# Apokleos/kata-xpu-device-plugin

Hardware: NVIDIA H100
Metric: pci.ids parse GB/s (x1000 text + 2^20-key join); device lookups/s reported beside it (higher is better)
Workload: dtype u8

## Files before the change

kata-xpu-device-plugin_b200/csrc/api.cu:

```cuda
#include <algorithm>
#include <cstdlib>
#include <new>
#include <vector>

#include "internal.cuh"
#include "pciids5.cu"
#include "finalize.cuh"
#include "small.cuh"
#include "scan.cuh"

void kx_exchange_destroy(kxpu_ctx *ctx);

static const char *kx_err_names[] = {
    "ok", "invalid argument", "CUDA error", "no sm_90 GPU available", "output buffer too small",
    "table capacity exceeded", "NCCL / peer exchange unavailable or failed", "input outside the supported domain", "out of memory"};

extern "C" const char *kxpu_strerror(int32_t status) {
    int i = -status;
    if (i < 0 || i > 8) return "unknown status";
    return kx_err_names[i];
}

extern "C" const char *kxpu_last_error(kxpu_ctx *ctx) {
    if (!ctx) return "null ctx";
// ... 293 lines not shown
    if (!t) return;
    if (t->arena.p) {
        if (ctx->pool.size() >= 4) {
            cudaStreamSynchronize(ctx->stream);
            cudaFree(ctx->pool.front().p);
            ctx->pool.erase(ctx->pool.begin());
        }
        arena_reset(ctx, t->arena);
        ctx->pool.push_back(t->arena);
    }
    delete t;
}

uint32_t kx_initial_blob_cap(kxpu_ctx *ctx, size_t n) {
    const uint32_t by_text = (uint32_t)std::min<size_t>(std::max<size_t>(n, 256), 4u << 20);
    return ctx->blob_hint > by_text ? ctx->blob_hint : by_text;
}

bool kx_grow_cap(uint32_t *cap, bool table_full) {
    if (*cap >= (1u << 28)) return false;
    const uint32_t sh = table_full ? 4u : 2u;
    *cap = (*cap >> (28u - sh)) ? (1u << 28) : (*cap << sh);
    return true;
}

void kx_note_table_size(kxpu_ctx *ctx, uint32_t nkeys, uint32_t blob_used, uint32_t blob_cap) {
    uint32_t ideal = 1u << 16;
    while (ideal < (1u << 28) && ideal / 2 < nkeys + nkeys / 8) ideal <<= 1;
    ctx->cap_hint = ideal;
    ctx->blob_hint = blob_cap > (4u << 20) && blob_used > (2u << 20) ? blob_cap : 0u;
}

int32_t kx_launch_parse(kxpu_ctx *ctx, kxpu_table *t, const uint8_t *d_text, size_t n, unsigned long long base,
                        unsigned long long carry_in, const KxXaHook *xa) {
    using namespace kxparse;
    const uint32_t num_chunks = (uint32_t)((n + CW - 1) / CW);
    kxparse5::Params5 P;
    memset(&P, 0, sizeof P);
    if (xa) { P.xa_on = 1; P.xa_done = xa->done; P.xa = xa->p; }
    if (num_chunks == 0) {
        if (xa) {
            P.tab = t->dev;
            P.task_ctas = 0;
            kxparse5::resolve_chunks_kernel<<<kxparse5::XA_CTAS, kxparse5::RES_WARPS * 32, 0, ctx->stream>>>(P);
            KX_LAUNCHED(ctx);
            KX_CUDA(ctx, cudaGetLastError());
        }
        return KXPU_OK;
    }
    P.text = d_text; P.n = n; P.base = base; P.num_chunks = num_chunks;
    P.tma_limit = n >= (size_t)STG_BYTES ? (uint32_t)((n - STG_BYTES) / CW) + 1u : 0u;
    static int per_sm = 0;
    const size_t smem = sizeof(kxparse5::WarpSmem5) * WARPS;
    if (per_sm == 0) {
        cudaOccupancyMaxActiveBlocksPerMultiprocessor(&per_sm, kxparse5::parse_kernel_v5, NT, smem);
        if (per_sm < 1) per_sm = 1;
    }
    const uint32_t wave_warps = (uint32_t)per_sm * ctx->sm_count * WARPS;
    P.rch = std::min<uint32_t>(std::max<uint32_t>(num_chunks / (wave_warps * 8u), 1u), kxparse5::RCH5_MAX);
    if (ctx->force_rch) P.rch = (uint32_t)ctx->force_rch;
    P.num_ranges = (num_chunks + P.rch - 1) / P.rch;
    P.range_state = t->range_words;
    P.range_carry = t->range_words + P.num_ranges;
    P.lead = (uint32_t *)(t->range_words + 2 * P.num_ranges);
    P.tasks = P.lead + P.num_ranges;
    P.tab = t->dev; P.carry_in = carry_in;
    uint32_t grid = (uint32_t)per_sm * ctx->sm_count;
    const uint32_t need = (P.num_ranges + WARPS - 1) / WARPS;
    if (grid > need) grid = need;
    {
        KxTimer tm(ctx, KXPU_T_PARSE);
        kxparse5::parse_kernel_v5<<<grid, NT, smem, ctx->stream>>>(P);
        KX_LAUNCHED(ctx);
    }
    {
        KxTimer tr(ctx, KXPU_T_RESOLVE);
        kxparse5::resolve_ranges_kernel<<<(P.num_ranges + 255u) / 256u, 256, 0, ctx->stream>>>(P);
        KX_LAUNCHED(ctx);
        const uint32_t rgrid = std::min<uint32_t>(4u * ctx->sm_count, (num_chunks + kxparse5::RES_WARPS - 1) / kxparse5::RES_WARPS);
        P.task_ctas = rgrid;
        kxparse5::resolve_chunks_kernel<<<rgrid + (xa ? kxparse5::XA_CTAS : 0u), kxparse5::RES_WARPS * 32, 0, ctx->stream>>>(P);
        KX_LAUNCHED(ctx);
    }
    KX_CUDA(ctx, cudaGetLastError());
    return KXPU_OK;
}

int32_t kx_launch_trunc(kxpu_ctx *ctx, kxpu_table *t, const uint8_t *d_text, size_t n, unsigned long long base) {
    kxparse::trunc_kernel<<<1, 1024, 0, ctx->stream>>>(d_text, n, base, t->dev.trunc, t->dev.counters);
    KX_LAUNCHED(ctx);
    KX_CUDA(ctx, cudaGetLastError());
    return KXPU_OK;
}

int32_t kx_launch_finalize(kxpu_ctx *ctx, kxpu_table *t, const uint8_t *d_text, size_t n, unsigned long long base,
                           const kxx::MinView *mv, const kxx::WaitSpec *wait, const KxSlabOut *slab) {
    kxparse::FinalizeParams F;
    memset(&F, 0, sizeof F);
    if (wait) F.wait = *wait;
    F.text = d_text; F.n = n; F.base = base; F.tab = t->dev;
    if (mv) F.mv = *mv;
    else { F.mv.a = t->dev.vendor_first; F.mv.stride = 0; F.mv.n = 1; F.mv.trunc1 = t->dev.trunc; }
    F.row_key = t->row_key; F.row_line = t->row_line; F.row_anchor = t->row_anchor;
    F.row_name_off = t->row_name_off; F.row_name_len = t->row_name_len;
    F.blob = t->blob; F.blob_cap = t->blob_cap;
    if (slab) {
        F.slab_rows = reinterpret_cast<kxx::SlabRow *>(slab->rows); F.slab_rows_cap = slab->rows_cap;
        F.blob = slab->blob; F.blob_cap = slab->blob_cap;
        F.tail = slab->tail;
    }
    KxTimer tm(ctx, KXPU_T_FINALIZE);
    F.scan_w = t->cap >= (1u << 19) ? 32u : 8u;
    if (ctx->force_scan_w) F.scan_w = (uint32_t)ctx->force_scan_w;
    const unsigned batches = (t->cap + 1 + F.scan_w - 1) / F.scan_w;
    const unsigned grid = std::min<unsigned>((batches + kxparse::SF_WARPS - 1) / kxparse::SF_WARPS, 8u * ctx->sm_count);
    kxparse::select_finalize_kernel<<<grid, kxparse::SF_WARPS * 32, 0, ctx->stream>>>(F);
    KX_LAUNCHED(ctx);
    KX_CUDA(ctx, cudaGetLastError());
    return KXPU_OK;
}

int32_t kx_launch_lookup(kxpu_ctx *ctx, kxpu_table *t, const uint32_t *d_keys, size_t n, int32_t *d_rows) {
    if (n == 0) return KXPU_OK;
    KxTimer tm(ctx, KXPU_T_LOOKUP);
    size_t blocks = (n + 255) / 256;
    size_t maxb = (size_t)ctx->sm_count * 32;
    if (blocks > maxb) blocks = maxb;
    kxparse::lookup_kernel<<<(unsigned)blocks, 256, 0, ctx->stream>>>(d_keys, n, t->dev.slots, t->cap, t->shift, d_rows);
    KX_LAUNCHED(ctx);
    KX_CUDA(ctx, cudaGetLastError());
    return KXPU_OK;
}

struct KxJoin {
    const uint32_t *d_keys;
    size_t n;
    int32_t *d_rows;
    int32_t *h_rows;
    const uint8_t *src_text;
};

static void *kx_mapped_host(const void *p) {
    if (!p) return nullptr;
    cudaPointerAttributes at;
    if (cudaPointerGetAttributes(&at, p) != cudaSuccess) { cudaGetLastError(); return nullptr; }
    return at.type == cudaMemoryTypeHost ? at.devicePointer : nullptr;
}

static uint32_t small_text_chunks(kxpu_ctx *ctx) {
    if (ctx->small_chunks < 0) {
        int coop = 0, per_sm = 0;
        cudaDeviceGetAttribute(&coop, cudaDevAttrCooperativeLaunch, ctx->device);
        cudaFuncSetAttribute(kxsmall::small_load_kernel, cudaFuncAttributeMaxDynamicSharedMemorySize, kxparse::WARPS * kxparse::STG_BYTES);
        cudaOccupancyMaxActiveBlocksPerMultiprocessor(&per_sm, kxsmall::small_load_kernel, kxparse::NT, kxparse::WARPS * kxparse::STG_BYTES);
        cudaGetLastError();
        ctx->small_chunks = (coop && !ctx->no_small) ? per_sm * ctx->sm_count * kxparse::WARPS : 0;
    }
    return (uint32_t)ctx->small_chunks;
}

static int32_t launch_small(kxpu_ctx *ctx, kxpu_table *t, const uint8_t *d_text, size_t n, const KxJoin *join) {
// ... 67 lines not shown
                    const long long t1 = tf[b * 8 + k], t0 = k ? tf[b * 8 + k - 1] : h[b * 8 + 4];
                    if (!t1 || !t0) continue;
                    const long long d = t1 - t0;
                    mn = std::min(mn, d); mx = std::max(mx, d); sum += d; cnt++;
                }
                if (cnt) fprintf(stderr, " %s %lld/%lld/%lld |", fn[k], mn, sum / cnt, mx);
            }
        }
        fprintf(stderr, "\n");
    }
    return KXPU_OK;
}

static int32_t kx_build_table_join(kxpu_ctx *ctx, const uint8_t *d_text, size_t n, kxpu_table **out, const KxJoin *join) {
    if ((reinterpret_cast<uintptr_t>(d_text) & 15u) != 0) {
        KX_SET_ERR(ctx, "device text pointer must be 16-byte aligned");
        return KXPU_E_INVALID;
    }
    if (n >= (1ull << 44)) return KXPU_E_UNSUPPORTED;
    uint32_t cap = ctx->cap_hint;
    while (cap > (1u << 16) && (size_t)cap / 2 > n / 6 + 1) cap >>= 1;
    uint32_t blob_cap = kx_initial_blob_cap(ctx, n);
    const uint32_t num_chunks = (uint32_t)((n + kxparse::CW - 1) / kxparse::CW);
    bool have_trunc = false;
    for (int attempt = 0; attempt < 12; attempt++) {
        kxpu_table *t = nullptr;
        int32_t rc = kx_table_acquire(ctx, cap, blob_cap, num_chunks, &t);
        if (rc != KXPU_OK) return rc;
        const bool small_path = num_chunks > 0 && num_chunks <= small_text_chunks(ctx) && !have_trunc;
        if (small_path) {
            rc = launch_small(ctx, t, d_text, n, join);
        } else {
            if (join && join->src_text && attempt == 0) cudaMemcpyAsync(const_cast<uint8_t *>(d_text), join->src_text, n, cudaMemcpyDefault, ctx->stream);
            rc = kx_launch_parse(ctx, t, d_text, n, 0, 0, nullptr);
            if (rc == KXPU_OK && have_trunc) rc = kx_launch_trunc(ctx, t, d_text, n, 0);
            if (rc == KXPU_OK) rc = kx_launch_finalize(ctx, t, d_text, n, 0, nullptr, nullptr, nullptr);
            if (rc == KXPU_OK && join) rc = kx_launch_lookup(ctx, t, join->d_keys, join->n, join->d_rows);
        }
        if (rc != KXPU_OK) { kx_table_release(ctx, t); return rc; }
        const bool zero_copy = small_path && join && join->src_text;
        if (!zero_copy) {
            if (join && join->h_rows && join->n) cudaMemcpyAsync(join->h_rows, join->d_rows, join->n * 4, cudaMemcpyDeviceToHost, ctx->stream);
            cudaMemcpyAsync(ctx->h_ctl, t->dev.counters, KX_C_COUNT * 4, cudaMemcpyDeviceToHost, ctx->stream);
        }
        cudaError_t e = cudaStreamSynchronize(ctx->stream);
        if (e != cudaSuccess) {
            KX_SET_ERR(ctx, "parse/finalize failed: %s", cudaGetErrorString(e));
            kx_table_release(ctx, t);
            return KXPU_E_CUDA;
        }
        const uint32_t *h = ctx->h_ctl;
        if (h[KX_C_OVERFLOW] || h[KX_C_NKEYS] > t->dev.max_keys) {
            kx_table_release(ctx, t);
            if (!kx_grow_cap(&cap, h[KX_C_OVERFLOW] != 0)) return KXPU_E_CAPACITY;
            continue;
        }
        if (h[KX_C_NEED_TRUNC] == 2u) {
            kx_table_release(ctx, t);
            have_trunc = true;
            continue;
        }
        if (h[KX_C_BLOB_OVERFLOW]) {
            kx_table_release(ctx, t);
            if ((size_t)blob_cap >= n) return KXPU_E_CAPACITY;
            blob_cap = (uint32_t)std::min<size_t>(std::max<size_t>(n, 256), (size_t)blob_cap * 8);
            continue;
        }
        t->n_rows = h[KX_C_NSEL];
        t->blob_used = h[KX_C_BLOB_CURSOR];
        kx_note_table_size(ctx, h[KX_C_NKEYS], t->blob_used, blob_cap);
        *out = t;
        return KXPU_OK;
    }
    return KXPU_E_CAPACITY;
}

// ... 187 lines not shown
```

kata-xpu-device-plugin_b200/csrc/common.cuh:

```cuda
#pragma once
#include <cuda_runtime.h>
#include <stdint.h>
#include <stdio.h>
#include <string.h>

#include <mutex>
#include <vector>

#include "../../include/kxpu.h"

constexpr int KX_MAX_RANKS = 16;


struct KxArena {
    void *p = nullptr;
    size_t bytes = 0;
    uint32_t cap = 0, blob_cap = 0;
    size_t range_bytes = 0;
};

struct KxExchange;
struct kxpu_multi;

struct kxpu_ctx {
    int device = -1;
    int sm_count = 0;
    cudaStream_t stream = nullptr;
    cudaEvent_t ev[2 * KXPU_T_COUNT] = {};
    cudaEvent_t ev_user[2] = {};
    bool ev_used[KXPU_T_COUNT] = {};
    int force_rch = 0;
    bool no_small = false;
    bool no_zero_copy = false;
    int force_scan_w = 0;
    int small_chunks = -1;
    bool stage_timing = true;
    uint64_t launches = 0;
    std::mutex mu;
    char err[512] = {0};
// ... 37 lines not shown
    void stop() {
        if (open) { cudaEventRecord(c->ev[2 * idx + 1], c->stream); c->ev_used[idx] = true; open = false; }
    }
    ~KxTimer() { stop(); }
};

static inline void kx_clear_timings(kxpu_ctx *c) { memset(c->ev_used, 0, sizeof(c->ev_used)); }

unsigned long long *kx_scan_state(kxpu_ctx *ctx, size_t words);
uint32_t kx_next_epoch(kxpu_ctx *ctx);

struct KxScratch {
    kxpu_ctx *c;
    std::vector<void *> ptrs;
    explicit KxScratch(kxpu_ctx *ctx) : c(ctx) {}
    cudaError_t alloc(void **p, size_t bytes) {
        cudaError_t e = cudaMallocAsync(p, bytes ? bytes : 16, c->stream);
        if (e == cudaSuccess) ptrs.push_back(*p);
        else *p = nullptr;
        return e;
    }
    ~KxScratch() {
        for (void *p : ptrs) cudaFreeAsync(p, c->stream);
    }
};

#ifdef __CUDACC__
__device__ __forceinline__ uint32_t kx_lane() { return threadIdx.x & 31u; }

__device__ __forceinline__ void kx_fence_gpu() { asm volatile("fence.acq_rel.gpu;" ::: "memory"); }
__device__ __forceinline__ void kx_fence_sys() { asm volatile("fence.acq_rel.sys;" ::: "memory"); }

__device__ __forceinline__ uint32_t kx_hash(uint32_t key) { return key * 0x9E3779B1u; }
#endif
```

kata-xpu-device-plugin_b200/csrc/finalize.cuh:

```cuda
#pragma once
#include "exchange.cuh"
#include "parse_common.cuh"

namespace kxparse {

constexpr unsigned long long MAX_TOKEN = 65536ull;

__global__ void __launch_bounds__(1024) trunc_kernel(const uint8_t *__restrict__ text, unsigned long long n,
                                                      unsigned long long base, unsigned long long *trunc_out, uint32_t *counters) {
    __shared__ unsigned long long s_first[1024], s_last[1024], s_bad[1024];
    const unsigned long long per = (n + 1023ull) / 1024ull;
    const unsigned long long lo = per * threadIdx.x, hi = lo + per < n ? lo + per : n;
    unsigned long long first = KX_NO_OFF, last = KX_NO_OFF, bad = KX_NO_OFF;
    for (unsigned long long i = lo; i < hi; i++) {
        if (text[i] == (uint8_t)'\n') {
            if (first == KX_NO_OFF) first = i;
            else if (i - last - 1 >= MAX_TOKEN && bad == KX_NO_OFF) bad = last + 1;
            last = i;
        }
    }
    s_first[threadIdx.x] = first; s_last[threadIdx.x] = last; s_bad[threadIdx.x] = bad;
    __syncthreads();
    if (threadIdx.x == 0) {
        unsigned long long prev_nl = KX_NO_OFF;
        unsigned long long res = KX_NO_OFF;
        for (int k = 0; k < 1024 && res == KX_NO_OFF; k++) {
            if (s_first[k] != KX_NO_OFF) {
                unsigned long long start = prev_nl == KX_NO_OFF ? 0 : prev_nl + 1;
                if (s_first[k] - start >= MAX_TOKEN) { res = start; break; }
                if (s_bad[k] != KX_NO_OFF) { res = s_bad[k]; break; }
                prev_nl = s_last[k];
            }
        }
        if (res == KX_NO_OFF) {
            unsigned long long start = prev_nl == KX_NO_OFF ? 0 : prev_nl + 1;
            if (n - start >= MAX_TOKEN) res = start;
        }
        *trunc_out = res == KX_NO_OFF ? KX_NO_OFF : base + res;
        counters[KX_C_NEED_TRUNC] = 1u;
    }
}

__device__ __forceinline__ bool is_re_space(uint32_t c) {
    return c == 0x20u || c == 0x09u || c == 0x0au || c == 0x0cu || c == 0x0du;
}
__device__ __forceinline__ uint32_t uspace_len(const uint8_t *s, uint32_t len) {
    if (len == 0) return 0;
    uint32_t c = s[0];
    if (c == 0x20u || (c >= 0x09u && c <= 0x0du)) return 1;
    if (len >= 2 && c == 0xC2u && (s[1] == 0x85u || s[1] == 0xA0u)) return 2;
    if (len >= 3) {
        uint32_t d = s[1], e = s[2];
        if (c == 0xE1u && d == 0x9Au && e == 0x80u) return 3;
        if (c == 0xE2u && d == 0x80u && ((e >= 0x80u && e <= 0x8Au) || e == 0xA8u || e == 0xA9u || e == 0xAFu)) return 3;
        if (c == 0xE2u && d == 0x81u && e == 0x9Fu) return 3;
// ... 16 lines not shown
    uint32_t c = buf[i];
    if (is_re_space(c)) return (i > start && is_re_space(buf[i - 1])) ? 0u : (uint32_t)'_';
    if (c >= 'a' && c <= 'z') return c - 32u;
    if (c == '/' || c == '.') return (uint32_t)'_';
    if ((c >= 'A' && c <= 'Z') || (c >= '0' && c <= '9') || c == '_') return c;
    if (i + 1 < end) {
        if (c == 0xC4u && buf[i + 1] == 0xB1u) return (uint32_t)'I';
        if (c == 0xC5u && buf[i + 1] == 0xBFu) return (uint32_t)'S';
    }
    return 0u;
}

constexpr int SF_WARPS = 8;
constexpr int SF_WIN = 128;
constexpr int SF_BATCH = 8;

struct FinalizeParams {
    const uint8_t *text;
    unsigned long long n, base;
    KxTableDev tab;
    kxx::MinView mv;
    uint32_t *row_key;
    unsigned long long *row_line;
    unsigned long long *row_anchor;
    uint32_t *row_name_off;
    uint32_t *row_name_len;
    uint8_t *blob;
    uint32_t blob_cap;
    kxx::WaitSpec wait;
    kxx::SlabRow *slab_rows;
    uint32_t slab_rows_cap;
    uint32_t scan_w;
    kxx::SlabTail tail;
    long long *trace;
};

__device__ __forceinline__ void finalize_store_row(const FinalizeParams &F, uint32_t row, uint32_t slot, uint32_t key, unsigned long long line,
                                                   unsigned long long anchor, uint32_t name_off, uint32_t name_len) {
    F.tab.slots[slot].row = (int32_t)row;
    if (F.slab_rows) {
        if (row < F.slab_rows_cap) {
            kxx::SlabRow r;
            r.key = key; r.name_len = name_len; r.line = line; r.anchor = anchor; r.name_off = name_off; r.pad = 0u;
            F.slab_rows[row] = r;
        }
    } else {
        F.row_key[row] = key; F.row_line[row] = line; F.row_anchor[row] = anchor;
        F.row_name_off[row] = name_off; F.row_name_len[row] = name_len;
    }
}

struct SfEntry {
    unsigned long long line, anchor;
    uint32_t slot, key;
};
constexpr int SF_QCAP = SF_BATCH - 1 + 32;

#define SF_MARK(k) do { if (F.trace && threadIdx.x == 0 && F.trace[blockIdx.x * 8u + (k)] == 0) F.trace[blockIdx.x * 8u + (k)] = clock64(); } while (0)

__device__ __forceinline__ void select_finalize_body(const FinalizeParams &F, const uint32_t scan_w) {
    __shared__ __align__(16) uint8_t s_raw[SF_WARPS][4][SF_WIN + 16];
    __shared__ uint8_t s_name[SF_WARPS][SF_BATCH][SF_WIN];
    __shared__ __align__(8) SfEntry s_q[SF_WARPS][SF_QCAP + 1];
    __shared__ uint32_t s_cnt[SF_WARPS], s_bytes[SF_WARPS], s_more[SF_WARPS], s_row0, s_blob0;
    if (F.tab.counters[KX_C_LONGLINE_HINT] != 0u && F.tab.counters[KX_C_NEED_TRUNC] != 1u) {
        if (blockIdx.x == 0 && threadIdx.x == 0) F.tab.counters[KX_C_NEED_TRUNC] = 2u;
// ... 221 lines not shown
                trim_space(g, len, start, end);
                for (uint32_t i = start; i < end; i++) out_len += sanitise_byte(g, i, start, end) != 0u;
                at = out_len ? atomicAdd(&F.tab.counters[KX_C_BLOB_CURSOR], out_len) : 0u;
                if (at + out_len > F.blob_cap) { F.tab.counters[KX_C_BLOB_OVERFLOW] = 1u; ok = false; }
                if (ok) {
                    uint32_t wr = at;
                    for (uint32_t i = start; i < end; i++) {
                        const uint32_t ch = sanitise_byte(g, i, start, end);
                        if (ch) F.blob[wr++] = (uint8_t)ch;
                    }
                }
            }
            if (lane == 0) finalize_store_row(F, row0 + r, l_slot, l_key, l_line, l_anchor, ok ? at : 0u, ok ? out_len : 0u);
            __syncwarp();
        }
        SF_MARK(5);
        {
            const uint32_t rem = qn - nvalid;
            if (nvalid != 0u && rem != 0u) {
                SfEntry e;
                if (lane < rem) e = q[nvalid + lane];
                __syncwarp();
                if (lane < rem) q[lane] = e;
                __syncwarp();
            }
            qn = rem;
        }
        __syncthreads();
        SF_MARK(6);
        if (!more) break;
    }
}

__global__ void __launch_bounds__(SF_WARPS * 32, 8) select_finalize_kernel(const FinalizeParams F) {
    kxx::wait_flags_cta(F.wait);
    select_finalize_body(F, F.scan_w);
    if (F.tail.on) {
        __syncthreads();
        if (threadIdx.x == 0) {
            kx_fence_sys();
            const uint32_t prev = atomicAdd(F.tail.done, 1u);
            if (prev == gridDim.x - 1u) {
                *F.tail.done = 0u;
                kx_fence_gpu();
                const volatile uint32_t *c = F.tab.counters;
                const uint32_t n_sel = c[KX_C_NSEL], blob_used = c[KX_C_BLOB_CURSOR];
                const bool over = c[KX_C_BLOB_OVERFLOW] || n_sel > F.tail.rows_cap || blob_used > F.tail.blob_cap;
                kxx::SlabHeader h;
                memset(&h, 0, sizeof h);
                h.n_rows = over ? 0u : n_sel;
                h.blob_bytes = over ? 0u : blob_used;
                h.status = over ? kxx::XS_SLAB_OVERFLOW : 0u;
                if (c[KX_C_OVERFLOW]) h.status |= kxx::XS_GROW | kxx::XS_FULL;
                if (c[KX_C_NKEYS] > F.tab.max_keys) h.status |= kxx::XS_GROW;
                h.nkeys = c[KX_C_NKEYS];
                *F.tail.header = h;
                kx_fence_sys();
                for (int k = 0; k < F.tail.tg.n; k++) *reinterpret_cast<volatile uint32_t *>(F.tail.tg.region[k] + F.tail.o_flag) = F.tail.epoch;
            }
        }
    }
}

__global__ void __launch_bounds__(256) lookup_kernel(const uint32_t *__restrict__ keys, size_t n, const KxSlot *__restrict__ slots,
                                                      uint32_t cap, uint32_t shift, int32_t *__restrict__ rows_out) {
    size_t i = (size_t)blockIdx.x * blockDim.x + threadIdx.x;
    const size_t stride = (size_t)gridDim.x * blockDim.x;
    for (; i < n; i += stride) rows_out[i] = table_probe(slots, cap, shift, keys[i]);
}

__global__ void __launch_bounds__(256) name_len_kernel(const int32_t *__restrict__ rows, size_t n,
                                                        const uint32_t *__restrict__ row_name_len, uint32_t n_rows,
                                                        uint32_t *__restrict__ lens) {
    size_t i = (size_t)blockIdx.x * blockDim.x + threadIdx.x;
    if (i < n) {
        int32_t r = rows[i];
        lens[i] = (r >= 0 && (uint32_t)r < n_rows) ? row_name_len[r] : 0u;
    }
}
__global__ void __launch_bounds__(256) name_copy_kernel(const int32_t *__restrict__ rows, size_t n,
                                                         const uint32_t *__restrict__ row_name_off,
                                                         const uint32_t *__restrict__ row_name_len, uint32_t n_rows,
                                                         const uint8_t *__restrict__ blob,
                                                         const uint32_t *__restrict__ offsets, uint8_t *__restrict__ out,
                                                         size_t cap) {
    size_t i = ((size_t)blockIdx.x * blockDim.x + threadIdx.x) >> 3;
    uint32_t sub = threadIdx.x & 7u;
    if (i >= n) return;
    int32_t r = rows[i];
    if (r < 0 || (uint32_t)r >= n_rows) return;
    uint32_t len = row_name_len[r], src = row_name_off[r], dst = offsets[i];
    if ((size_t)dst + len > cap) return;
    for (uint32_t k = sub; k < len; k += 8u) out[dst + k] = blob[src + k];
}

__global__ void __launch_bounds__(256) arena_reset_kernel(uint4 *ff, size_t n_ff16, uint32_t *counters) {
    const size_t i = (size_t)blockIdx.x * blockDim.x + threadIdx.x;
    const size_t stride = (size_t)gridDim.x * blockDim.x;
// ... 6 lines not shown
```

kata-xpu-device-plugin_b200/csrc/internal.cuh:

```cuda
#pragma once
#include "common.cuh"
#include "exchange.cuh"
#include "table.cuh"

struct kxpu_table {
    uint32_t cap = 0, shift = 0;
    KxArena arena;
    KxTableDev dev{};
    unsigned long long *range_words = nullptr;
    uint32_t *row_key = nullptr;
    unsigned long long *row_line = nullptr;
    unsigned long long *row_anchor = nullptr;
    uint32_t *row_name_off = nullptr;
    uint32_t *row_name_len = nullptr;
    uint32_t *sel = nullptr;
    uint8_t *blob = nullptr;
    uint32_t blob_cap = 0;
    uint32_t rows_cap = 0;
    uint32_t n_rows = 0;
    uint32_t blob_used = 0;
};

#define KX_ENTER(ctx)                          \
    if (!(ctx)) return KXPU_E_INVALID;         \
    std::lock_guard<std::mutex> guard__((ctx)->mu); \
    cudaSetDevice((ctx)->device)

int32_t kx_table_acquire(kxpu_ctx *ctx, uint32_t cap, uint32_t blob_cap, uint32_t num_chunks, kxpu_table **out);
void kx_table_release(kxpu_ctx *ctx, kxpu_table *t);
uint32_t kx_initial_blob_cap(kxpu_ctx *ctx, size_t n);
struct KxXaHook {
    kxx::XaParams p;
    uint32_t *done;
};
int32_t kx_launch_parse(kxpu_ctx *ctx, kxpu_table *t, const uint8_t *d_text, size_t n, unsigned long long base,
                        unsigned long long carry_in, const KxXaHook *xa);
int32_t kx_launch_trunc(kxpu_ctx *ctx, kxpu_table *t, const uint8_t *d_text, size_t n, unsigned long long base);
struct KxSlabOut {
    uint8_t *rows;
    uint32_t rows_cap;
    uint8_t *blob;
    uint32_t blob_cap;
    kxx::SlabTail tail;
};
int32_t kx_launch_finalize(kxpu_ctx *ctx, kxpu_table *t, const uint8_t *d_text, size_t n, unsigned long long base,
                           const kxx::MinView *mv, const kxx::WaitSpec *wait, const KxSlabOut *slab);
int32_t kx_launch_lookup(kxpu_ctx *ctx, kxpu_table *t, const uint32_t *d_keys, size_t n, int32_t *d_rows);
bool kx_grow_cap(uint32_t *cap, bool table_full);
void kx_note_table_size(kxpu_ctx *ctx, uint32_t nkeys, uint32_t blob_used, uint32_t blob_cap);
```

kata-xpu-device-plugin_b200/csrc/pciids5.cu:

```cuda
#pragma once
#include "exchange.cuh"
#include "parse_common.cuh"

namespace kxparse5 {

using namespace kxparse;

constexpr int STAGES5 = 3;
constexpr int RCH5_MAX = 8;
constexpr int RES_WARPS = 8;

struct WarpSmem5 {
    alignas(16) uint8_t stage[STAGES5][STG_BYTES];
    alignas(8) unsigned long long bar[STAGES5];
};

struct Params5 {
    const uint8_t *text;
    unsigned long long n, base;
    uint32_t num_chunks;
    uint32_t tma_limit;
    uint32_t rch;
    uint32_t num_ranges;
    unsigned long long *range_state;
    uint32_t *lead;
    unsigned long long *range_carry;
    uint32_t *tasks;
    KxTableDev tab;
    unsigned long long carry_in;
    uint32_t task_ctas;
    int xa_on;
    uint32_t *xa_done;
    kxx::XaParams xa;
};


__device__ __forceinline__ void nl_masks(uint32_t st, uint32_t lane, uint32_t n_rel, uint32_t k7f, uint32_t k0a, uint32_t k80,
                                         uint32_t (&nl)[2], uint32_t &rawnl) {
    const uint32_t swz = (lane >> 2) & 1u;
    rawnl = 0;
#pragma unroll
    for (int h = 0; h < 2; h++) {
        const uint32_t o = (uint32_t)h * HALF + lane * 32u;
        const uint4 va = lds128(st + o + 16u * swz);
        const uint4 vb = lds128(st + o + 16u * (swz ^ 1u));
        const uint32_t ma = nl_mask16(va, k7f, k0a, k80), mb = nl_mask16(vb, k7f, k0a, k80);
        const uint32_t m2 = ma | (mb << 16);
        uint32_t mm = __funnelshift_l(m2, m2, swz << 4);
        rawnl |= mm;
        if (n_rel <= (uint32_t)CW) mm &= n_rel > o + 1u ? (n_rel - o - 1u >= 32u ? 0xffffffffu : ((1u << (n_rel - o - 1u)) - 1u)) : 0u;
        nl[h] = mm;
    }
}

// ... 17 lines not shown
        const uint32_t c0 = lds8(lp0 + (31u - (uint32_t)__clz((int)b0)));
        const uint32_t c1 = lds8(lp0 + (uint32_t)HALF + (31u - (uint32_t)__clz((int)b1)));
        if (c0 != 9u && c0 != 35u) t0 |= b0;
        if (c1 != 9u && c1 != 35u) t1 |= b1;
    }
}

__device__ __forceinline__ uint32_t devs_of(uint32_t lp, uint32_t mm) {
    uint32_t km = 0;
    while (mm) {
        const uint32_t bit = mm & (0u - mm);
        mm ^= bit;
        const uint32_t a = lp + (31u - (uint32_t)__clz((int)bit));
        if (lds8(a) == 9u && lds8(a + 1u) != 9u) km |= bit;
    }
    return km;
}

__global__ void __launch_bounds__(NT, 4) parse_kernel_v5(const Params5 P) {
    extern __shared__ __align__(128) uint8_t smem_raw[];
    WarpSmem5 *W = reinterpret_cast<WarpSmem5 *>(smem_raw);
    uint32_t lane = threadIdx.x & 31u;
    const uint32_t w = threadIdx.x >> 5;
    asm volatile("" : "+r"(lane));
    const uint32_t lt_mask = (1u << lane) - 1u;

    if (lane == 0) {
        for (int s = 0; s < STAGES5; s++) mbar_init(&W[w].bar[s], 1);
        asm volatile("fence.mbarrier_init.release.cluster;" ::: "memory");
    }
    uint32_t tk = 0;
    if (lane == 0) tk = atomicAdd(&P.tab.counters[KX_C_TICKET], 1u);
    uint32_t r = __shfl_sync(0xffffffffu, tk, 0);
    if (r >= P.num_ranges) return;

    uint32_t a_stage0 = smem_u32(smem_raw) + w * (uint32_t)sizeof(WarpSmem5);
    asm volatile("" : "+r"(a_stage0));
    const uint32_t a_bar0 = a_stage0 + (uint32_t)offsetof(WarpSmem5, bar);

    uint32_t k7f = 0x7f7f7f7fu, k0a = 0x0a0a0a0au, k80 = 0x80808080u;
    asm volatile("" : "+r"(k7f), "+r"(k0a), "+r"(k80));

    const unsigned long long pol = l2_evict_first_policy();
    auto issue = [&](uint32_t g, uint32_t s) {
        if (g < P.tma_limit) {
            mbar_expect_tx_a(a_bar0 + 8u * s, STG_BYTES);
            tma_load_a(a_stage0 + s * (uint32_t)STG_BYTES, P.text + (unsigned long long)g * CW, STG_BYTES, a_bar0 + 8u * s, pol);
        }
    };
    const uint32_t rch = P.rch;
    bool staged = false;

    uint32_t phase_bits = 0, s = 0;
    uint32_t nfresh = 0;
    for (;;) {
        uint32_t tk2 = 0, r_next = 0xffffffffu;
        bool have_next = false;
        if (lane == 0) tk2 = atomicAdd(&P.tab.counters[KX_C_TICKET], 1u);
        uint32_t rc_x = 0, rc_g = 0;
        if (r == 0u) {
            rc_x = LS_PUB | (((P.carry_in & CV_HAS_TOP) && (P.carry_in & CV_VOK)) ? (LS_TOP | LS_VOK) : 0u);
            rc_g = 0xffffffffu;
        }
        uint32_t lead = r == 0u ? 0u : rch;
        const bool table_dead = *reinterpret_cast<volatile uint32_t *>(&P.tab.counters[KX_C_OVERFLOW]) != 0u;
        const uint32_t gb = r * rch;
        const uint32_t cnt = P.num_chunks - gb < rch ? P.num_chunks - gb : rch;
        if (!staged && lane == 0) {
            for (uint32_t j = 0; j < (uint32_t)STAGES5 && j < cnt; j++) issue(gb + j, (s + j) % (uint32_t)STAGES5);
        }
        staged = false;
        for (uint32_t i = 0; i < cnt; i++) {
            if (!have_next && rch > (uint32_t)STAGES5 && i + (uint32_t)STAGES5 >= rch) {
                r_next = __shfl_sync(0xffffffffu, tk2, 0);
                have_next = true;
            }
            const uint32_t g = gb + i;
            const uint32_t st = a_stage0 + s * (uint32_t)STG_BYTES;
            const unsigned long long cbase = P.base + (unsigned long long)g * CW;
            uint32_t n_rel = CW + 1;
            if (g < P.tma_limit) {
                const uint32_t bar = a_bar0 + 8u * s, par = (phase_bits >> s) & 1u;
                while (!mbar_try_a(bar, par)) {
                }
                phase_bits ^= 1u << s;
            } else {
                n_rel = stage_chunk_manual(P.text, P.n, g, lane, W[w].stage[s]);
            }

            uint32_t nl[2], th[2], rawnl;
            nl_masks(st, lane, n_rel, k7f, k0a, k80, nl, rawnl);
            tops_of2(st + lane * 32u + 1u, nl[0], nl[1], th[0], th[1]);

            uint32_t linfo0 = P_NONE, linfo1 = P_NONE;
            bool any_alive = (g == 0u) || (rc_x & LS_VOK) != 0u;
            {
                uint32_t t0 = th[0], t1 = th[1];
                while (t0 | t1) {
                    const bool second = t0 == 0u;
                    const uint32_t tmv = second ? t1 : t0;
                    const uint32_t bit = tmv & (0u - tmv);
                    if (second) t1 = tmv ^ bit; else t0 = tmv ^ bit;
                    const uint32_t p = (second ? (uint32_t)HALF : 0u) + lane * 32u + 1u + (31u - (uint32_t)__clz((int)bit));
                    uint32_t val;
                    const bool ok = hex4_swar(lds32_unaligned(st + p), val);
                    const unsigned long long line_g = cbase + p;
                    bool alive = ok;
                    if (ok) {
                        const unsigned long long vf = P.tab.vendor_first[val];
                        if (line_g < vf) atomicMin(&P.tab.vendor_first[val], line_g);
                        alive = line_g <= vf;
                    }
                    any_alive |= alive;
                    const uint32_t info = (alive ? 0x80000000u : 0u) | ((ok ? val : 0u) << 15) | p;
                    if (second) linfo1 = info; else linfo0 = info;
                }
            }
            const uint32_t bal0 = __ballot_sync(0xffffffffu, th[0] != 0u);
// ... 91 lines not shown
            if ((bal0 | bal1) == 0u && n_rel > (uint32_t)CW && __reduce_or_sync(0xffffffffu, rawnl) == 0u && lane == 0)
                atomicOr(&P.tab.counters[KX_C_LONGLINE_HINT], 1u);

            __syncwarp();
            {
                const uint32_t fi = i + (uint32_t)STAGES5;
                uint32_t fg = 0xffffffffu;
                if (fi < rch) {
                    fg = g + (uint32_t)STAGES5;
                } else if (rch > (uint32_t)STAGES5 && cnt == rch && r_next < P.num_ranges) {
                    fg = r_next * rch + (fi - rch);
                    staged = true;
                }
                if (lane == 0) issue(fg, s);
            }
            s = s == (uint32_t)STAGES5 - 1u ? 0u : s + 1u;
        }
        if (lane == 0) {
            unsigned long long v = ST_NONE;
            if (rc_x != 0u) {
                if (rc_g == 0xffffffffu)
                    v = ST_PREFIX | P.carry_in;
                else
                    v = ST_PREFIX | CV_HAS_TOP | ((rc_x & LS_VOK) ? CV_VOK : 0ull) | ((unsigned long long)((rc_x >> 12) & 0xffffu) << 44) |
                        ((P.base + (unsigned long long)rc_g * CW + (rc_x & 0xfffu)) & CV_ANCHOR_MASK);
            }
            P.range_state[r] = v;
            P.lead[r] = lead < cnt ? lead : cnt;
        }
        if (!have_next) r_next = __shfl_sync(0xffffffffu, tk2, 0);
        r = r_next;
        if (r >= P.num_ranges) break;
    }
}

constexpr uint32_t XA_CTAS = 64;

__global__ void __launch_bounds__(256) resolve_ranges_kernel(const Params5 P) {
    const uint32_t rr = blockIdx.x * blockDim.x + threadIdx.x;
    const uint32_t lane = threadIdx.x & 31u;
    const uint32_t rr0 = rr - lane;
    if (rr0 >= P.num_ranges) return;
    const bool live = rr < P.num_ranges;
    const uint32_t nlead = live ? P.lead[rr] : 0u;
    const unsigned long long own = live ? P.range_state[rr] : ST_NONE;
    const uint32_t pm = __ballot_sync(0xffffffffu, (own & ST_MASK) == ST_PREFIX);
    const uint32_t below = pm & ((1u << lane) - 1u);
    const unsigned long long from_warp = __shfl_sync(0xffffffffu, own, below ? 31 - __clz((int)below) : 0);
    unsigned long long warp_in = 0;
    const uint32_t first_p = pm ? (uint32_t)__ffs((int)pm) - 1u : 32u;
    const bool want = __any_sync(0xffffffffu, nlead != 0u && lane <= first_p);
    if (want) {
        long long q0 = (long long)rr0 - 32;
        for (;;) {
            const long long q = q0 + lane;
            const unsigned long long sv = q >= 0 ? P.range_state[q] : (q == -1 ? (ST_PREFIX | P.carry_in) : ST_NONE);
            const uint32_t m = __ballot_sync(0xffffffffu, (sv & ST_MASK) == ST_PREFIX);
            if (m) {
                warp_in = __shfl_sync(0xffffffffu, sv, 31 - __clz((int)m));
                break;
            }
            q0 -= 32;
        }
    }
    const unsigned long long carry = (below ? from_warp : warp_in) & ~ST_MASK;
    const bool alive = nlead != 0u && (carry & CV_HAS_TOP) && (carry & CV_VOK) &&
                       P.tab.vendor_first[(uint32_t)(carry >> 44) & 0xffffu] >= (carry & CV_ANCHOR_MASK);
    const uint32_t mine = alive ? nlead : 0u;
    uint32_t incl = mine;
#pragma unroll
    for (int d = 1; d < 32; d <<= 1) {
        const uint32_t y = __shfl_up_sync(0xffffffffu, incl, d);
        if (lane >= (uint32_t)d) incl += y;
    }
// ... 6 lines not shown
    const uint32_t at = at0 + incl - mine;
    for (uint32_t j = 0; j < nlead; j++) P.tasks[at + j] = rr * P.rch + j;
}

__global__ void __launch_bounds__(RES_WARPS * 32) resolve_chunks_kernel(const Params5 P) {
    __shared__ __align__(16) uint8_t stg[RES_WARPS][STG_BYTES];
    __shared__ __align__(8) unsigned long long bars[RES_WARPS];
    __shared__ uint16_t plist[RES_WARPS][704];
    if (blockIdx.x >= P.task_ctas) {
        kxx::xa_push_slice(P.xa, (blockIdx.x - P.task_ctas) * blockDim.x + threadIdx.x, XA_CTAS * blockDim.x);
        __syncthreads();
        if (threadIdx.x == 0) {
            kx_fence_sys();
            const uint32_t prev = atomicAdd(P.xa_done, 1u);
            if (prev == XA_CTAS - 1u) {
                *P.xa_done = 0u;
                kx_fence_sys();
                kxx::xa_finish(P.xa);
            }
        }
        return;
    }
    const uint32_t lane = threadIdx.x & 31u, w = threadIdx.x >> 5;
    const uint32_t lt_mask = (1u << lane) - 1u;
    uint32_t k7f = 0x7f7f7f7fu, k0a = 0x0a0a0a0au, k80 = 0x80808080u;
    asm volatile("" : "+r"(k7f), "+r"(k0a), "+r"(k80));
    const uint32_t st = smem_u32(stg[w]), bar = smem_u32(&bars[w]);
    if (lane == 0) {
        mbar_init(&bars[w], 1);
        asm volatile("fence.mbarrier_init.release.cluster;" ::: "memory");
    }
    __syncwarp();
    const unsigned long long pol = l2_evict_first_policy();
    const uint32_t n_tasks = P.tab.counters[KX_C_DEFER];
    uint32_t par = 0, nfresh = 0;
    const bool small_tab = P.tab.cap <= (1u << 20);
    uint32_t it = 0;
    for (uint32_t t = blockIdx.x * RES_WARPS + w; t < n_tasks; t += P.task_ctas * RES_WARPS, it++) {
        if ((it & 3u) == 0u && *reinterpret_cast<volatile uint32_t *>(&P.tab.counters[KX_C_OVERFLOW]) != 0u) break;
        const uint32_t gg = P.tasks[t];
        uint32_t n_rel = CW + 1;
        if (gg < P.tma_limit) {
            if (lane == 0) {
                mbar_expect_tx_a(bar, STG_BYTES);
                tma_load_a(st, P.text + (unsigned long long)gg * CW, STG_BYTES, bar, pol);
            }
            while (!mbar_try_a(bar, par)) {
            }
            par ^= 1u;
        } else {
            n_rel = stage_chunk_manual(P.text, P.n, gg, lane, stg[w]);
        }
        const unsigned long long cc = P.range_carry[gg / P.rch];
        const uint32_t key_hi = ((uint32_t)(cc >> 44) & 0xffffu) << 16;
        const unsigned long long anchor = cc & CV_ANCHOR_MASK;
        uint32_t kh[2], th[2], rawnl;
        chunk_masks(st, lane, n_rel, k7f, k0a, k80, kh, th, rawnl);
        const uint32_t bal0 = __ballot_sync(0xffffffffu, th[0] != 0u);
        const uint32_t bal1 = __ballot_sync(0xffffffffu, th[1] != 0u);
        const uint32_t pre0 = kh[0] & ~th[0] & (th[0] ? (th[0] & (0u - th[0])) - 1u : 0xffffffffu);
        const uint32_t pre1 = kh[1] & ~th[1] & (th[1] ? (th[1] & (0u - th[1])) - 1u : 0xffffffffu);
        const unsigned long long cbase = P.base + (unsigned long long)gg * CW;
        const uint32_t m0 = (bal0 & lt_mask) == 0u ? pre0 : 0u;
        const uint32_t m1 = (bal0 == 0u && (bal1 & lt_mask) == 0u) ? pre1 : 0u;
        const uint32_t mine = (uint32_t)__popc(m0) + (uint32_t)__popc(m1);
        uint32_t incl = mine;
// ... 36 lines not shown
```

kata-xpu-device-plugin_b200/csrc/table.cuh:

```cuda
#pragma once
#include "common.cuh"

#define KX_EMPTY_KEY 0xFFFFFFFFu
#define KX_NO_OFF 0xFFFFFFFFFFFFFFFFull

#define KX_C_TICKET 0
#define KX_C_DEFER 1
#define KX_C_GRIDBAR 2
#define KX_C_NKEYS 32
#define KX_C_NSEL 33
#define KX_C_BLOB_CURSOR 64
#define KX_C_OVERFLOW 96
#define KX_C_LONGLINE_HINT 97
#define KX_C_NROWS 98
#define KX_C_BLOB_OVERFLOW 99
#define KX_C_NEED_TRUNC 100
#define KX_C_XSTATUS 101
#define KX_C_XROWS 102
#define KX_C_XBLOB 103
#define KX_C_XMAXKEYS 104
#define KX_C_COUNT 128

struct __align__(32) KxSlot {
    uint32_t key;
    int32_t row;
    unsigned long long min_line;
    unsigned long long min_anchor;
    unsigned long long spare;
};

struct KxTableDev {
    KxSlot *slots;
    unsigned long long *vendor_first;
    uint32_t *counters;
    unsigned long long *trunc;
    uint32_t cap;
    uint32_t shift;
    uint32_t max_keys;
};
```

Measured before the change: 2536.

## Chain parse pipeline kernels with programmatic dependent launch and fold counter readback

Launches resolve, trunc, finalize and lookup kernels with programmatic stream serialization and adds griddepcontrol wait/launch_dependents calls, so each kernel's launch and prologue can overlap the tail of the previous one. It also removes the separate device-to-host counter memcpy on the large path. Instead the last finalize CTA, or block 0 of the lookup kernel, writes the counters directly to mapped host memory. The risk is correctness of the early release points and of host visibility of the counters, plus extra atomics in finalize.

```diff
diff --git a/kata-xpu-device-plugin_b200/csrc/api.cu b/kata-xpu-device-plugin_b200/csrc/api.cu
--- a/kata-xpu-device-plugin_b200/csrc/api.cu
+++ b/kata-xpu-device-plugin_b200/csrc/api.cu
@@ -349,7 +349,7 @@
 }
 
 int32_t kx_launch_parse(kxpu_ctx *ctx, kxpu_table *t, const uint8_t *d_text, size_t n, unsigned long long base,
-                        unsigned long long carry_in, const KxXaHook *xa) {
+                        unsigned long long carry_in, const KxXaHook *xa, bool chained) {
     using namespace kxparse;
     const uint32_t num_chunks = (uint32_t)((n + CW - 1) / CW);
     kxparse5::Params5 P;
@@ -392,26 +392,26 @@
     }
     {
         KxTimer tr(ctx, KXPU_T_RESOLVE);
-        kxparse5::resolve_ranges_kernel<<<(P.num_ranges + 255u) / 256u, 256, 0, ctx->stream>>>(P);
+        KX_CUDA(ctx, kx_launch(ctx, chained, kxparse5::resolve_ranges_kernel, (P.num_ranges + 255u) / 256u, 256, 0, P));
         KX_LAUNCHED(ctx);
         const uint32_t rgrid = std::min<uint32_t>(4u * ctx->sm_count, (num_chunks + kxparse5::RES_WARPS - 1) / kxparse5::RES_WARPS);
         P.task_ctas = rgrid;
-        kxparse5::resolve_chunks_kernel<<<rgrid + (xa ? kxparse5::XA_CTAS : 0u), kxparse5::RES_WARPS * 32, 0, ctx->stream>>>(P);
+        KX_CUDA(ctx, kx_launch(ctx, chained, kxparse5::resolve_chunks_kernel, rgrid + (xa ? kxparse5::XA_CTAS : 0u), kxparse5::RES_WARPS * 32, 0, P));
         KX_LAUNCHED(ctx);
     }
     KX_CUDA(ctx, cudaGetLastError());
     return KXPU_OK;
 }
 
-int32_t kx_launch_trunc(kxpu_ctx *ctx, kxpu_table *t, const uint8_t *d_text, size_t n, unsigned long long base) {
-    kxparse::trunc_kernel<<<1, 1024, 0, ctx->stream>>>(d_text, n, base, t->dev.trunc, t->dev.counters);
+int32_t kx_launch_trunc(kxpu_ctx *ctx, kxpu_table *t, const uint8_t *d_text, size_t n, unsigned long long base, bool chained) {
+    KX_CUDA(ctx, kx_launch(ctx, chained, kxparse::trunc_kernel, 1, 1024, 0, d_text, (unsigned long long)n, base, t->dev.trunc, t->dev.counters));
     KX_LAUNCHED(ctx);
     KX_CUDA(ctx, cudaGetLastError());
     return KXPU_OK;
 }
 
 int32_t kx_launch_finalize(kxpu_ctx *ctx, kxpu_table *t, const uint8_t *d_text, size_t n, unsigned long long base,
-                           const kxx::MinView *mv, const kxx::WaitSpec *wait, const KxSlabOut *slab) {
+                           const kxx::MinView *mv, const kxx::WaitSpec *wait, const KxSlabOut *slab, bool chained, uint32_t *h_ctl) {
     kxparse::FinalizeParams F;
     memset(&F, 0, sizeof F);
     if (wait) F.wait = *wait;
@@ -426,24 +426,26 @@
         F.blob = slab->blob; F.blob_cap = slab->blob_cap;
         F.tail = slab->tail;
     }
+    F.h_ctl = h_ctl;
     KxTimer tm(ctx, KXPU_T_FINALIZE);
     F.scan_w = t->cap >= (1u << 19) ? 32u : 8u;
     if (ctx->force_scan_w) F.scan_w = (uint32_t)ctx->force_scan_w;
     const unsigned batches = (t->cap + 1 + F.scan_w - 1) / F.scan_w;
     const unsigned grid = std::min<unsigned>((batches + kxparse::SF_WARPS - 1) / kxparse::SF_WARPS, 8u * ctx->sm_count);
-    kxparse::select_finalize_kernel<<<grid, kxparse::SF_WARPS * 32, 0, ctx->stream>>>(F);
+    KX_CUDA(ctx, kx_launch(ctx, chained, kxparse::select_finalize_kernel, grid, kxparse::SF_WARPS * 32, 0, F));
     KX_LAUNCHED(ctx);
     KX_CUDA(ctx, cudaGetLastError());
     return KXPU_OK;
 }
 
-int32_t kx_launch_lookup(kxpu_ctx *ctx, kxpu_table *t, const uint32_t *d_keys, size_t n, int32_t *d_rows) {
+int32_t kx_launch_lookup(kxpu_ctx *ctx, kxpu_table *t, const uint32_t *d_keys, size_t n, int32_t *d_rows, bool chained, uint32_t *h_ctl) {
     if (n == 0) return KXPU_OK;
     KxTimer tm(ctx, KXPU_T_LOOKUP);
     size_t blocks = (n + 255) / 256;
     size_t maxb = (size_t)ctx->sm_count * 32;
     if (blocks > maxb) blocks = maxb;
-    kxparse::lookup_kernel<<<(unsigned)blocks, 256, 0, ctx->stream>>>(d_keys, n, t->dev.slots, t->cap, t->shift, d_rows);
+    KX_CUDA(ctx, kx_launch(ctx, chained, kxparse::lookup_kernel, (unsigned)blocks, 256, 0, d_keys, n, (const KxSlot *)t->dev.slots, t->cap,
+                           t->shift, d_rows, (const uint32_t *)t->dev.counters, h_ctl));
     KX_LAUNCHED(ctx);
     KX_CUDA(ctx, cudaGetLastError());
     return KXPU_OK;
@@ -577,16 +579,18 @@
             rc = launch_small(ctx, t, d_text, n, join);
         } else {
             if (join && join->src_text && attempt == 0) cudaMemcpyAsync(const_cast<uint8_t *>(d_text), join->src_text, n, cudaMemcpyDefault, ctx->stream);
-            rc = kx_launch_parse(ctx, t, d_text, n, 0, 0, nullptr);
-            if (rc == KXPU_OK && have_trunc) rc = kx_launch_trunc(ctx, t, d_text, n, 0);
-            if (rc == KXPU_OK) rc = kx_launch_finalize(ctx, t, d_text, n, 0, nullptr, nullptr, nullptr);
-            if (rc == KXPU_OK && join) rc = kx_launch_lookup(ctx, t, join->d_keys, join->n, join->d_rows);
+            const bool chained = !ctx->stage_timing;
+            rc = kx_launch_parse(ctx, t, d_text, n, 0, 0, nullptr, chained);
+            if (rc == KXPU_OK && have_trunc) rc = kx_launch_trunc(ctx, t, d_text, n, 0, chained);
+            const bool joins = join && join->n;
+            if (rc == KXPU_OK) rc = kx_launch_finalize(ctx, t, d_text, n, 0, nullptr, nullptr, nullptr, chained, joins ? nullptr : ctx->h_ctl);
+            if (rc == KXPU_OK && joins) rc = kx_launch_lookup(ctx, t, join->d_keys, join->n, join->d_rows, chained, ctx->h_ctl);
         }
         if (rc != KXPU_OK) { kx_table_release(ctx, t); return rc; }
         const bool zero_copy = small_path && join && join->src_text;
         if (!zero_copy) {
             if (join && join->h_rows && join->n) cudaMemcpyAsync(join->h_rows, join->d_rows, join->n * 4, cudaMemcpyDeviceToHost, ctx->stream);
-            cudaMemcpyAsync(ctx->h_ctl, t->dev.counters, KX_C_COUNT * 4, cudaMemcpyDeviceToHost, ctx->stream);
+            if (small_path) cudaMemcpyAsync(ctx->h_ctl, t->dev.counters, KX_C_COUNT * 4, cudaMemcpyDeviceToHost, ctx->stream);
         }
         cudaError_t e = cudaStreamSynchronize(ctx->stream);
         if (e != cudaSuccess) {
diff --git a/kata-xpu-device-plugin_b200/csrc/common.cuh b/kata-xpu-device-plugin_b200/csrc/common.cuh
--- a/kata-xpu-device-plugin_b200/csrc/common.cuh
+++ b/kata-xpu-device-plugin_b200/csrc/common.cuh
@@ -5,6 +5,7 @@
 #include <string.h>
 
 #include <mutex>
+#include <utility>
 #include <vector>
 
 #include "../../include/kxpu.h"
@@ -108,4 +109,23 @@
 __device__ __forceinline__ void kx_fence_sys() { asm volatile("fence.acq_rel.sys;" ::: "memory"); }
 
 __device__ __forceinline__ uint32_t kx_hash(uint32_t key) { return key * 0x9E3779B1u; }
+
+__device__ __forceinline__ void kx_grid_wait() { asm volatile("griddepcontrol.wait;" ::: "memory"); }
+__device__ __forceinline__ void kx_grid_release() { asm volatile("griddepcontrol.launch_dependents;" ::: "memory"); }
 #endif
+
+template <typename... KArgs, typename... Args>
+static inline cudaError_t kx_launch(kxpu_ctx *ctx, bool chained, void (*kernel)(KArgs...), unsigned grid, unsigned block, size_t smem,
+                                    Args &&...args) {
+    cudaLaunchAttribute at[1];
+    at[0].id = cudaLaunchAttributeProgrammaticStreamSerialization;
+    at[0].val.programmaticStreamSerializationAllowed = 1;
+    cudaLaunchConfig_t cfg = {};
+    cfg.gridDim = dim3(grid);
+    cfg.blockDim = dim3(block);
+    cfg.dynamicSmemBytes = smem;
+    cfg.stream = ctx->stream;
+    cfg.attrs = at;
+    cfg.numAttrs = chained ? 1 : 0;
+    return cudaLaunchKernelEx(&cfg, kernel, std::forward<Args>(args)...);
+}
diff --git a/kata-xpu-device-plugin_b200/csrc/finalize.cuh b/kata-xpu-device-plugin_b200/csrc/finalize.cuh
--- a/kata-xpu-device-plugin_b200/csrc/finalize.cuh
+++ b/kata-xpu-device-plugin_b200/csrc/finalize.cuh
@@ -21,6 +21,8 @@
     }
     s_first[threadIdx.x] = first; s_last[threadIdx.x] = last; s_bad[threadIdx.x] = bad;
     __syncthreads();
+    kx_grid_wait();
+    kx_grid_release();
     if (threadIdx.x == 0) {
         unsigned long long prev_nl = KX_NO_OFF;
         unsigned long long res = KX_NO_OFF;
@@ -103,6 +105,7 @@
     uint32_t slab_rows_cap;
     uint32_t scan_w;
     kxx::SlabTail tail;
+    uint32_t *h_ctl;
     long long *trace;
 };
 
@@ -390,9 +393,29 @@
     }
 }
 
+__device__ __forceinline__ void counters_to_host(const uint32_t *counters, uint32_t *h_ctl) {
+    if (threadIdx.x < KX_C_COUNT) h_ctl[threadIdx.x] = __ldcg(&counters[threadIdx.x]);
+}
+
 __global__ void __launch_bounds__(SF_WARPS * 32, 8) select_finalize_kernel(const FinalizeParams F) {
+    kx_grid_wait();
+    kx_grid_release();
     kxx::wait_flags_cta(F.wait);
     select_finalize_body(F, F.scan_w);
+    if (F.h_ctl) {
+        __shared__ uint32_t s_last;
+        __syncthreads();
+        if (threadIdx.x == 0) {
+            kx_fence_gpu();
+            s_last = atomicAdd(&F.tab.counters[KX_C_FIN_DONE], 1u) == gridDim.x - 1u;
+            if (s_last) {
+                F.tab.counters[KX_C_FIN_DONE] = 0u;
+                kx_fence_gpu();
+            }
+        }
+        __syncthreads();
+        if (s_last) counters_to_host(F.tab.counters, F.h_ctl);
+    }
     if (F.tail.on) {
         __syncthreads();
         if (threadIdx.x == 0) {
@@ -421,7 +444,10 @@
 }
 
 __global__ void __launch_bounds__(256) lookup_kernel(const uint32_t *__restrict__ keys, size_t n, const KxSlot *__restrict__ slots,
-                                                      uint32_t cap, uint32_t shift, int32_t *__restrict__ rows_out) {
+                                                      uint32_t cap, uint32_t shift, int32_t *__restrict__ rows_out,
+                                                      const uint32_t *counters, uint32_t *h_ctl) {
+    kx_grid_wait();
+    if (h_ctl && blockIdx.x == 0) counters_to_host(counters, h_ctl);
     size_t i = (size_t)blockIdx.x * blockDim.x + threadIdx.x;
     const size_t stride = (size_t)gridDim.x * blockDim.x;
     for (; i < n; i += stride) rows_out[i] = table_probe(slots, cap, shift, keys[i]);
diff --git a/kata-xpu-device-plugin_b200/csrc/internal.cuh b/kata-xpu-device-plugin_b200/csrc/internal.cuh
--- a/kata-xpu-device-plugin_b200/csrc/internal.cuh
+++ b/kata-xpu-device-plugin_b200/csrc/internal.cuh
@@ -34,8 +34,8 @@
     uint32_t *done;
 };
 int32_t kx_launch_parse(kxpu_ctx *ctx, kxpu_table *t, const uint8_t *d_text, size_t n, unsigned long long base,
-                        unsigned long long carry_in, const KxXaHook *xa);
-int32_t kx_launch_trunc(kxpu_ctx *ctx, kxpu_table *t, const uint8_t *d_text, size_t n, unsigned long long base);
+                        unsigned long long carry_in, const KxXaHook *xa, bool chained = false);
+int32_t kx_launch_trunc(kxpu_ctx *ctx, kxpu_table *t, const uint8_t *d_text, size_t n, unsigned long long base, bool chained = false);
 struct KxSlabOut {
     uint8_t *rows;
     uint32_t rows_cap;
@@ -44,7 +44,9 @@
     kxx::SlabTail tail;
 };
 int32_t kx_launch_finalize(kxpu_ctx *ctx, kxpu_table *t, const uint8_t *d_text, size_t n, unsigned long long base,
-                           const kxx::MinView *mv, const kxx::WaitSpec *wait, const KxSlabOut *slab);
-int32_t kx_launch_lookup(kxpu_ctx *ctx, kxpu_table *t, const uint32_t *d_keys, size_t n, int32_t *d_rows);
+                           const kxx::MinView *mv, const kxx::WaitSpec *wait, const KxSlabOut *slab, bool chained = false,
+                           uint32_t *h_ctl = nullptr);
+int32_t kx_launch_lookup(kxpu_ctx *ctx, kxpu_table *t, const uint32_t *d_keys, size_t n, int32_t *d_rows, bool chained = false,
+                         uint32_t *h_ctl = nullptr);
 bool kx_grow_cap(uint32_t *cap, bool table_full);
 void kx_note_table_size(kxpu_ctx *ctx, uint32_t nkeys, uint32_t blob_used, uint32_t blob_cap);
diff --git a/kata-xpu-device-plugin_b200/csrc/pciids5.cu b/kata-xpu-device-plugin_b200/csrc/pciids5.cu
--- a/kata-xpu-device-plugin_b200/csrc/pciids5.cu
+++ b/kata-xpu-device-plugin_b200/csrc/pciids5.cu
@@ -103,7 +103,10 @@
     uint32_t tk = 0;
     if (lane == 0) tk = atomicAdd(&P.tab.counters[KX_C_TICKET], 1u);
     uint32_t r = __shfl_sync(0xffffffffu, tk, 0);
-    if (r >= P.num_ranges) return;
+    if (r >= P.num_ranges) {
+        kx_grid_release();
+        return;
+    }
 
     uint32_t a_stage0 = smem_u32(smem_raw) + w * (uint32_t)sizeof(WarpSmem5);
     asm volatile("" : "+r"(a_stage0));
@@ -312,6 +315,7 @@
         r = r_next;
         if (r >= P.num_ranges) break;
     }
+    kx_grid_release();
 }
 
 constexpr uint32_t XA_CTAS = 64;
@@ -320,6 +324,8 @@
     const uint32_t rr = blockIdx.x * blockDim.x + threadIdx.x;
     const uint32_t lane = threadIdx.x & 31u;
     const uint32_t rr0 = rr - lane;
+    kx_grid_wait();
+    kx_grid_release();
     if (rr0 >= P.num_ranges) return;
     const bool live = rr < P.num_ranges;
     const uint32_t nlead = live ? P.lead[rr] : 0u;
@@ -392,6 +398,8 @@
     }
     __syncwarp();
     const unsigned long long pol = l2_evict_first_policy();
+    kx_grid_wait();
+    kx_grid_release();
     const uint32_t n_tasks = P.tab.counters[KX_C_DEFER];
     uint32_t par = 0, nfresh = 0;
     const bool small_tab = P.tab.cap <= (1u << 20);
diff --git a/kata-xpu-device-plugin_b200/csrc/table.cuh b/kata-xpu-device-plugin_b200/csrc/table.cuh
--- a/kata-xpu-device-plugin_b200/csrc/table.cuh
+++ b/kata-xpu-device-plugin_b200/csrc/table.cuh
@@ -7,6 +7,7 @@
 #define KX_C_TICKET 0
 #define KX_C_DEFER 1
 #define KX_C_GRIDBAR 2
+#define KX_C_FIN_DONE 3
 #define KX_C_NKEYS 32
 #define KX_C_NSEL 33
 #define KX_C_BLOB_CURSOR 64
```

Result: no change. 2559, median of 6 (+0.9%).

## Load only chunk body via TMA and fill trailing overlap from next stage

Applied to the files above, without the earlier changes.

Each TMA load now copies just CW bytes per chunk instead of CW+TRAIL, so the overlapping tail is not fetched twice from global memory. The tail is filled by copying the first 16 bytes of the next staged chunk in shared memory, falling back to a second TMA or to scalar global loads at range ends. Stage buffers are padded to a 128-byte stride. In exchange the warp now waits on the next stage's barrier earlier and adds an extra shared-memory copy plus a syncwarp per chunk.

```diff
diff --git a/kata-xpu-device-plugin_b200/csrc/api.cu b/kata-xpu-device-plugin_b200/csrc/api.cu
--- a/kata-xpu-device-plugin_b200/csrc/api.cu
+++ b/kata-xpu-device-plugin_b200/csrc/api.cu
@@ -367,6 +367,7 @@
     }
     P.text = d_text; P.n = n; P.base = base; P.num_chunks = num_chunks;
     P.tma_limit = n >= (size_t)STG_BYTES ? (uint32_t)((n - STG_BYTES) / CW) + 1u : 0u;
+    P.body_limit = (uint32_t)(n / CW);
     static int per_sm = 0;
     const size_t smem = sizeof(kxparse5::WarpSmem5) * WARPS;
     if (per_sm == 0) {
diff --git a/kata-xpu-device-plugin_b200/csrc/pciids5.cu b/kata-xpu-device-plugin_b200/csrc/pciids5.cu
--- a/kata-xpu-device-plugin_b200/csrc/pciids5.cu
+++ b/kata-xpu-device-plugin_b200/csrc/pciids5.cu
@@ -10,8 +10,9 @@
 constexpr int RCH5_MAX = 8;
 constexpr int RES_WARPS = 8;
 
+constexpr uint32_t STG_STRIDE5 = (STG_BYTES + 127) & ~127;
 struct WarpSmem5 {
-    alignas(16) uint8_t stage[STAGES5][STG_BYTES];
+    alignas(128) uint8_t stage[STAGES5][STG_STRIDE5];
     alignas(8) unsigned long long bar[STAGES5];
 };
 
@@ -20,6 +21,7 @@
     unsigned long long n, base;
     uint32_t num_chunks;
     uint32_t tma_limit;
+    uint32_t body_limit;
     uint32_t rch;
     uint32_t num_ranges;
     unsigned long long *range_state;
@@ -114,9 +116,13 @@
 
     const unsigned long long pol = l2_evict_first_policy();
     auto issue = [&](uint32_t g, uint32_t s) {
-        if (g < P.tma_limit) {
-            mbar_expect_tx_a(a_bar0 + 8u * s, STG_BYTES);
-            tma_load_a(a_stage0 + s * (uint32_t)STG_BYTES, P.text + (unsigned long long)g * CW, STG_BYTES, a_bar0 + 8u * s, pol);
+        if (g < P.body_limit) {
+            const uint32_t dst = a_stage0 + s * STG_STRIDE5, bar = a_bar0 + 8u * s;
+            const unsigned long long src = (unsigned long long)g * CW;
+            const bool tr = ((g + 1u) % P.rch == 0u) && src + CW + TRAIL <= P.n;
+            mbar_expect_tx_a(bar, tr ? (uint32_t)STG_BYTES : (uint32_t)CW);
+            tma_load_a(dst, P.text + src, CW, bar, pol);
+            if (tr) tma_load_a(dst + CW, P.text + src + CW, TRAIL, bar, pol);
         }
     };
     const uint32_t rch = P.rch;
@@ -147,14 +153,29 @@
                 have_next = true;
             }
             const uint32_t g = gb + i;
-            const uint32_t st = a_stage0 + s * (uint32_t)STG_BYTES;
+            const uint32_t st = a_stage0 + s * STG_STRIDE5;
             const unsigned long long cbase = P.base + (unsigned long long)g * CW;
             uint32_t n_rel = CW + 1;
-            if (g < P.tma_limit) {
+            if (g < P.body_limit) {
                 const uint32_t bar = a_bar0 + 8u * s, par = (phase_bits >> s) & 1u;
                 while (!mbar_try_a(bar, par)) {
                 }
                 phase_bits ^= 1u << s;
+                const unsigned long long nx = (unsigned long long)(g + 1u) * CW;
+                n_rel = CW + (nx < P.n ? 1u : 0u);
+                const bool last = i + 1u == cnt;
+                if (!last && g + 1u < P.body_limit) {
+                    const uint32_t s1 = s == (uint32_t)STAGES5 - 1u ? 0u : s + 1u;
+                    while (!mbar_try_a(a_bar0 + 8u * s1, (phase_bits >> s1) & 1u)) {
+                    }
+                    if (lane == 0) {
+                        const uint4 v = lds128(a_stage0 + s1 * STG_STRIDE5);
+                        asm volatile("st.shared.v4.u32 [%0], {%1, %2, %3, %4};" ::"r"(st + CW), "r"(v.x), "r"(v.y), "r"(v.z), "r"(v.w) : "memory");
+                    }
+                } else if ((!last || nx + TRAIL > P.n) && lane < (uint32_t)TRAIL) {
+                    asm volatile("st.shared.u8 [%0], %1;" ::"r"(st + CW + lane), "r"(nx + lane < P.n ? (uint32_t)P.text[nx + lane] : 0u) : "memory");
+                }
+                __syncwarp();
             } else {
                 n_rel = stage_chunk_manual(P.text, P.n, g, lane, W[w].stage[s]);
             }
```

New measurement: 2527 before, 2602 after, median of 6. 1.03x the previous value.
